# navigator8972/vae_assoc

Measured on AMD Instinct MI355X. Metric: paired-samples/sec (img+jnt assoc-VAE train step), higher is better.
Workload: dtype bf16

## Files before the change

### vae_assoc_amd/csrc/avae_device.h

```cpp
#pragma once
#include <hip/hip_runtime.h>
#include <stdint.h>

namespace avae {

constexpr int kMaxMod = 4;
constexpr int kThreads = 256;
constexpr int kTileBytesK = 128;
constexpr int kRowAlign = 256;
constexpr int kLatentRows = 16;
constexpr int kAdamRows = 16;
constexpr int kCostHist = 4096;

enum Kind : int {
    K_FWD_HIDDEN = 0,
    K_FWD_HEAD = 1,
    K_FWD_OUT_LOSS = 2,
    K_FWD_OUT_STORE = 3,
    K_DGRAD_HIDDEN = 4,
    K_DGRAD_LATENT = 5,
    K_WGRAD = 6,
    K_DGRAD_F32 = 10,
    K_LATENT = 7,
    K_COST = 8,
// ... 28 lines not shown
    void* out2;
    const void* aux0;
    const void* aux1;
    const void* aux2;
    float* partial;
    const float* eps;
    float wts[kMaxMod];
    const void* tail_w;
    void* tail_out;
    const void* tail_aux;
    int tail_mode;
    int tail_n;
    int tail_ldw, tail_ldo, tail_ldx;
    int tail_act;
    int tail_kt;
    int conv;
    const unsigned char* present;
    int present_ld;
};

struct ConvA {
    const void* src;
    const void* consts;
    int M, K;
    int OHW, OW, IH, IW, Cin;
    int k, so, d, pad;
    int src_sb, src_sp;
    int ones;
    unsigned mg_ohw, mg_ow, mg_k, mg_cin;
};
// ... 32 lines not shown
struct TnLaunchArgs {
    int n_items;
    int grid_x;
    int xcd_group;
    int sched;
    int adam;
    long long d_theta, d_m, d_v;
    float beta1, beta2, eps;
    const DevState* st;
    const ConvA* conv_tab;
    int xcd_pieces;
    TnPiece pieces[8][kTnPieces];
    TnItem items[kMaxTnItems];
};
static_assert(sizeof(TnLaunchArgs) <= 4096, "kernel arguments are passed by value: 4 KiB");

struct DevState {
    long long step;
    float last_cost;
    float lr_t;
    float cost_hist[kCostHist];
};

struct AdamItem {
    float* theta;
    float* m;
    float* v;
    const float* g;
    void* W;
    void* Wt;
// ... 216 lines not shown
int tile_lds_bytes(int tile_cfg, bool two_c_tiles);
void launch_grouped(int compute_dtype, int tile_cfg, const LaunchArgs& args, int grid_x, int grid_y, int lds_bytes,
                    DevState* st, hipStream_t s, unsigned long long* stamps = nullptr, int launch_id = 0);
void launch_grouped_tn(int compute_dtype, int tile_cfg, const TnLaunchArgs& args, int grid_x, int grid_y, int lds_bytes,
                       DevState* st, hipStream_t s, unsigned long long* stamps = nullptr, int launch_id = 0);
void launch_adam(int compute_dtype, const AdamArgs& a, int n_blocks, hipStream_t s);
void launch_prep(int compute_dtype, const PrepArgs& a, hipStream_t s);
const void* prep_kernel(int compute_dtype, bool masked);
void launch_fill(void* base, int elem_bytes, unsigned bits, long long start, long long stride, int count, hipStream_t s);
void launch_sums(const ReduceArgs& a, int n_blocks, hipStream_t s);
int small_head_lds_bytes();
void launch_small_latb(int compute_dtype, int act, const LaunchArgs& args, int grid_x, int grid_y, int lds_bytes, DevState* st, hipStream_t s,
                       unsigned long long* stamps, int launch_id);
void launch_small_head(int compute_dtype, int act, const LaunchArgs& args, int grid_x, int grid_y, int lds_bytes, hipStream_t s,
                       unsigned long long* stamps, int launch_id);
void launch_small_tn(int compute_dtype, const TnLaunchArgs& args, int grid_x, int grid_y, hipStream_t s, unsigned long long* stamps, int launch_id);
void launch_small_loss(int compute_dtype, const LaunchArgs& args, int grid_x, int grid_y, int lds_bytes, hipStream_t s, unsigned long long* stamps, int launch_id);
void launch_small(int compute_dtype, const LaunchArgs& args, int grid_x, int grid_y, int lds_bytes, hipStream_t s, unsigned long long* stamps, int launch_id);
void launch_reduce(const ReduceArgs& a, int n_blocks, hipStream_t s);
void launch_chain2(int compute_dtype, const LaunchArgs& args, int grid_x, int grid_y, int lds_bytes, unsigned* counters, unsigned* err, hipStream_t s);

}
```

### vae_assoc_amd/csrc/avae_host.hip

```cpp
#include "avae_device.h"
#include "avae_complete.h"
#include "../../include/avae.h"

#include <dlfcn.h>
#include <sched.h>
#include <unistd.h>

#include <algorithm>
#include <cmath>
#include <cstdio>
#include <cstdlib>
#include <cstring>
#include <functional>
#include <map>
#include <mutex>
#include <stdexcept>
#include <string>
#include <vector>

using namespace avae;

namespace {

thread_local std::string g_create_error;
// ... 154 lines not shown
    size_t P_flat = 0, P_int = 0, P_enc = 0;
    size_t off_theta = 0, off_m = 0, off_v = 0, off_g = 0;
    size_t stage_lo = 0, stage_bytes = 0;
    size_t off_eps = 0, off_partial = 0, off_state = 0, off_items = 0, off_adam = 0, off_inf = 0, off_stamps = 0, off_latent = 0;
    int n_partial = 0;
    size_t ws_bytes = 0;
    unsigned char* ws = nullptr;
    bool own_ws = false;
    hipStream_t cap_stream = nullptr;

    std::vector<WorkItem> items;
    std::vector<Launch> bwd;
    std::vector<Launch> wgrad;
    std::vector<Launch> wgrad_adam;
    int n_buckets = 1;
    int bwd_split = 0;
    std::vector<Launch> wgrad_b[2];
    struct Range { size_t off, count; };
    std::vector<Range> ranges_b[2];
    int adam_first_b[2] = {0, 0}, adam_count_b[2] = {0, 0}, adam_blocks_b[2] = {0, 0};
    std::vector<AdamItem> adam_items_b;
    size_t off_adam_b = 0;
    void* comm = nullptr;
    int comm_world = 1, comm_rank = 0;
    bool comm_on = false;
    size_t off_wire = 0;
    unsigned char* ipc_block = nullptr;
    size_t ipc_bytes = 0;
    unsigned char* ipc_peer[kMaxWorld] = {nullptr, nullptr, nullptr, nullptr, nullptr, nullptr, nullptr, nullptr};
    bool ipc_opened[kMaxWorld] = {false, false, false, false, false, false, false, false};
// ... 941 lines not shown
            bool lean = true;
            int act = -1;
            for (int k = 0; k < Lp.count; ++k) {
                const WorkItem& n = h->items[Lp.first + k];
                if (n.kind == K_COST) continue;
                lean = lean && n.kind == want_p && n.tail_mode == mode
                            && (act < 0 || act == n.tail_act) && n.K > 0 && 2 * n.nz <= 64 && n.tail_kt >= 1 && n.tail_kt <= 2;
                act = n.tail_act;
            }
            if (lean && mode == 1)
                for (int k = 0; k < Lp.count; ++k) lean = lean && h->items[Lp.first + k].kind == K_FWD_HEAD && h->items[Lp.first + k].out1 != nullptr;
            if (lean) { Lp.cfg = mode == 2 ? 10 : 11; Lp.lds = small_head_lds_bytes(); Lp.lean_act = act; }
        }
        return true;
    };
    auto every_conv = [](const Mod&) { return true; };
    auto gather_launch = [&](const std::string& name, std::vector<Launch>& dst, auto&& stage_of, auto&& src_of, auto&& want) {
        Launch L;
        L.name = name; L.type = 1;
        int base = 0;
        for (Mod& md : h->mods) if (md.conv && want(md)) {
            GatherSeg g = bd.gather_seg(stage_of(md), src_of(md));
            g.tile_base = base; base += g.tiles_r * g.tiles_c;
            L.ga.seg[L.ga.n_seg++] = g;
        }
        L.blocks = base;
        if (base > 0) dst.push_back(L);
    };
    auto col2im_launch = [&](const std::string& name, std::vector<Launch>& dst, auto&& stage_of, auto&& prev_of, auto&& want) {
        Launch L;
// ... 60 lines not shown
                      [&](Mod& md) { return h->at<void>(md.cenc[2].Y.rm); }, [](const Mod& md) { return !md.cenc[3].impl; });
    }
    group("fwd_head", h->plain.fwd, [&] { for (Mod& md : h->mods) h->items.push_back(bd.fwd_head(md, true, md.conv && md.cenc[3].impl)); });
    bool latent_alone = false;
    {
        long t64 = 0, t128 = 0;
        bool narrow = false;
        for (const Mod& md : h->mods) {
            t64 += (long)((h->B + 255) / 256) * ((md.n_in + 63) / 64);
            t128 += (long)((h->B + 127) / 128) * ((md.n_in + 127) / 128);
            narrow = narrow || md.n_in <= 64 || h->B <= 64;
        }
        latent_alone = t64 >= 192 && t128 >= 192 && !narrow && !std::getenv("AVAE_NO_LOSS8");
    }
    if (latent_alone) group("latent", h->plain.fwd, [&] { h->items.push_back(bd.latent()); });
    for (int k = 0; k < std::max(Lmax, 1); ++k) {
        group("fwd_dec" + std::to_string(k + 1), h->plain.fwd, [&] {
            for (Mod& md : h->mods) if (k < md.L) h->items.push_back(bd.fwd_hidden(k == 0 ? md.Z : md.D[k - 1], md.dec[k], md.D[k]));
        });
        if (k == 0 && !any_conv && !latent_alone) fuse_tail(h->plain.fwd, 1);
    }
    if (any_conv) {
        Launch L;
        L.name = "conv_wadj"; L.type = 6;
        int base = 0;
        for (Mod& md : h->mods) if (md.conv) for (const ConvStage& st : md.cdec) if (st.adj) {
            WadjSeg& g = L.wa.seg[L.wa.n_seg++];
            g.Wt = h->at<void>(st.d.Wt); g.Wadj = h->at<void>(st.Wadj); g.Wf = h->at<void>(st.Wf); g.ldt = st.d.ldt; g.ldadj = st.ldadj; g.ldf = st.ldf;
            g.k = st.g.k; g.Cin = st.g.Cin; g.Cout = st.d.out;
            g.block_base = base; base += (st.g.Cin * st.g.k * st.g.k * st.d.out + kThreads - 1) / kThreads;
        }
        L.blocks = base;
        if (base > 0 && std::getenv("AVAE_NO_WADJ_FOLD")) h->plain.fwd.push_back(L);
    }
    if (any_conv) {
// ... 84 lines not shown
            if (!md.conv) h->items.push_back(bd.dgrad_latent(md));
            else if (md.cdec[0].impl_bwd) h->items.push_back(bd.adj_dgrad_latent_impl(md.cdec[0], md));
        }
        h->items.push_back(bd.cost(true));
    });
    (void)latent_conv_impl;
    h->bwd_split = (int)h->bwd.size();
    group("bwd_head", h->bwd, [&] {
        for (Mod& md : h->mods) {
            if (md.conv && md.cenc[3].impl_bwd)
                h->items.push_back(bd.adj_dgrad_impl(md.cenc[3], h->at<void>(md.dH.rm), md.dH.ld, md.dH.ld, md.cenc[2].act, md.cenc[2].Y, md.cenc[2].dY));
            else if (md.conv) h->items.push_back(bd.conv_dgrad(md.cenc[3], md.dH));
            else h->items.push_back(bd.dgrad_hidden(md.dH, md.head, md.E.back(), md.dE.back()));
        }
    });
    if (!any_conv) fuse_tail(h->bwd, 2);
    if (any_conv) {
        for (int i = 3; i >= 1; --i) {
            col2im_launch("conv_enc" + std::to_string(i) + "_col2im", h->bwd, [&](Mod& md) -> const ConvStage& { return md.cenc[i]; },
                          [&](Mod& md) -> const ConvStage* { return &md.cenc[i - 1]; }, [i](const Mod& md) { return !md.cenc[i].impl_bwd; });
            if (i >= 2) group("conv_bwd_enc" + std::to_string(i), h->bwd, [&] {
                for (Mod& md : h->mods) if (md.conv) {
                    const ConvStage& st = md.cenc[i - 1];
                    if (st.impl_bwd) h->items.push_back(bd.adj_dgrad_impl(st, h->at<void>(st.dY.rm), st.g.OH * st.g.OW * st.dY.ld, st.dY.ld, md.cenc[i - 2].act, md.cenc[i - 2].Y, md.cenc[i - 2].dY));
                    else h->items.push_back(bd.conv_dgrad(st, st.dY));
                } });
        }
    }
    for (int k = Lmax - 1; k >= 1; --k) {
        group("bwd_enc" + std::to_string(k + 1), h->bwd, [&] {
            for (Mod& md : h->mods) if (k < md.L) h->items.push_back(bd.dgrad_hidden(md.dE[k], md.enc[k], md.E[k - 1], md.dE[k - 1]));
        });
    }
    if (any_conv && !std::getenv("AVAE_NO_SINK")) {
        auto plain_kind = [](int k) { return k == K_FWD_HIDDEN || k == K_DGRAD_HIDDEN || k == K_DGRAD_F32; };
        std::vector<const void*> conv_bufs;
        for (const Mod& md : h->mods) if (md.conv) {
            for (const Act* a : {&md.Z, &md.dH, &md.dO}) conv_bufs.push_back(h->at<void>(a->rm));
            for (const std::vector<ConvStage>* side : {&md.cenc, &md.cdec})
                for (const ConvStage& st : *side) { conv_bufs.push_back(h->at<void>(st.Y.rm)); conv_bufs.push_back(h->at<void>(st.dY.rm)); }
        }
        auto mlp_item = [&](const WorkItem& w) {
            if (w.conv > 0) return false;
            for (const void* q : conv_bufs) if (q == w.out0 || q == w.A) return false;
            return true;
        };
        auto reads = [&](const Launch& L, const std::vector<const void*>& outs) {
            if (L.type != 0) return false;
// ... 439 lines not shown
    return L;
}

void run_launch(avae_handle* h, const Launch& L, hipStream_t s, unsigned long long* stamps, int stamp) {
    Timed t(h, s, L.name);
    if (L.type == 1) launch_gather(h->cfg.compute_dtype, L.ga, L.blocks, s);
    else if (L.type == 2) launch_col2im(h->cfg.compute_dtype, L.ca, L.blocks, s);
    else if (L.type == 3) launch_reduce(L.ra, L.blocks, s);
    else if (L.type == 4) launch_thin(h->cfg.compute_dtype, L.ta, L.blocks, s);
    else if (L.type == 5) launch_colsum(L.ra, L.blocks, s);
    else if (L.type == 6) launch_wadj(h->cfg.compute_dtype, L.wa, L.blocks, s);
    else if (L.type == 7) launch_gperm(L.gp, L.blocks, s);
    else if (L.type == 8) launch_rowsum(h->cfg.compute_dtype, L.rs, L.blocks, s);
    else if (L.type == 9) launch_sums(L.ra, L.blocks, s);
    else if (L.cfg == 13) launch_chain2(h->cfg.compute_dtype, L.args, L.grid_x, L.grid_y, L.lds, h->at<unsigned>(h->off_chain), h->at<unsigned>(h->off_chain) + kMaxMod * 64, s);
    else if (L.cfg == 11) launch_small_head(h->cfg.compute_dtype, L.lean_act, L.args, L.grid_x, L.grid_y, L.lds, s, stamps, stamp);
    else if (L.cfg == 10) launch_small_latb(h->cfg.compute_dtype, L.lean_act, L.args, L.grid_x, L.grid_y, L.lds, h->state(), s, stamps, stamp);
    else if (L.cfg == 9) launch_small_loss(h->cfg.compute_dtype, L.args, L.grid_x, L.grid_y, L.lds, s, stamps, stamp);
    else if (L.cfg == 7) launch_small(h->cfg.compute_dtype, L.args, L.grid_x, L.grid_y, L.lds, s, stamps, stamp);
    else if (L.tn && L.cfg == 12) launch_small_tn(h->cfg.compute_dtype, L.targs, L.grid_x, L.grid_y, s, stamps, stamp);
    else if (L.tn) launch_grouped_tn(h->cfg.compute_dtype, L.cfg, L.targs, L.grid_x, L.grid_y, L.lds, h->state(), s, stamps, stamp);
    else launch_grouped(h->cfg.compute_dtype, L.cfg, L.args, L.grid_x, L.grid_y, L.lds, h->state(), s, stamps, stamp);
    LAUNCH_OK(L.name);
    if (h->debug_sync) {
        std::fprintf(stderr, "[avae] launch %s type=%d cfg=%d items=%d blocks=%d\n", L.name.c_str(), L.type, L.cfg, L.count, L.blocks);
        for (int i = 0; i < L.args.n_items && L.type == 0; ++i)
            std::fprintf(stderr, "        item kind=%d M=%d N=%d K=%d lda=%d ldb=%d tiles=%dx%d\n", L.args.items[i].kind, L.args.items[i].M,
                         L.args.items[i].N, L.args.items[i].K, L.args.items[i].lda, L.args.items[i].ldb, L.args.items[i].tiles_m, L.args.items[i].tiles_n);
        for (int i = 0; i < L.ga.n_seg && L.type == 1; ++i)
            std::fprintf(stderr, "        gather B=%d IH=%d Cin=%d OH=%d k=%d so=%d d=%d pad=%d sb=%d sp=%d ones=%d ldp=%d tiles=%dx%d\n", L.ga.seg[i].g.B, L.ga.seg[i].g.IH,
// ... 396 lines not shown
    bool any_conv = false;
    for (const Mod& md : h->mods) any_conv = any_conv || md.conv;
    out[0].clear(); out[1].clear();
    if (any_conv || h->cfg.comm_buckets == 1) { *n_buckets = 1; out[0].push_back({0, h->P_int + 1}); return; }
    *n_buckets = 2;
    out[1].push_back({0, h->P_enc});
    out[0].push_back({h->P_enc, h->P_int + 1 - h->P_enc});
}

void dp_segment(avae_handle* h, int j, int bucket, hipStream_t s, bool direct = false) {
    if (bucket < 0 || bucket >= h->n_buckets) throw Err("data-parallel bucket out of range");
    if (j < 0 || j >= kMultiSteps) throw Err("staging set out of range");
    auto body = [&](hipStream_t cs) {
        auto run = [&](const std::vector<Launch>& ls, size_t lo, size_t hi) { run_set(h, ls, lo, hi, j, cs); };
        if (h->n_buckets == 1) { run(h->plain.fwd, 0, h->plain.fwd.size()); run(h->bwd, 0, h->bwd.size()); run(h->wgrad, 0, h->wgrad.size()); return; }
        if (bucket == 0) { run(h->plain.fwd, 0, h->plain.fwd.size()); run(h->bwd, 0, (size_t)h->bwd_split); run(h->wgrad_b[0], 0, h->wgrad_b[0].size()); }
        else { run(h->bwd, (size_t)h->bwd_split, h->bwd.size()); run(h->wgrad_b[1], 0, h->wgrad_b[1].size()); }
    };
    if (h->cfg.use_graph && !h->timing && !direct) {
        if (h->g_dp[bucket].empty()) h->g_dp[bucket].resize(kMultiSteps);
        if (!h->g_dp[bucket][j].exec) h->g_dp[bucket][j] = capture(h, body);
        HIP_OK(hipGraphLaunch(h->g_dp[bucket][j].exec, s));
    } else {
        body(s);
    }
}

void dp_allreduce(avae_handle* h, int b, hipStream_t cs) {
    const avae_handle::Range& r = h->ranges_b[b][0];
    float* g = h->grad();
    const bool has_cost = r.off + r.count == h->P_int + 1;
    const size_t n = has_cost ? r.count - 1 : r.count;
// ... 1223 lines not shown
```

### vae_assoc_amd/csrc/avae_kernels.hip

```cpp
#include "avae_device.h"
#include "avae_complete.h"
#include <hip/hip_ext.h>
#include <stdexcept>
#include "../../include/avae.h"

namespace avae {

typedef __attribute__((ext_vector_type(8))) __bf16 bf16x8;
typedef __attribute__((ext_vector_type(4))) __bf16 bf16x4;
typedef __attribute__((ext_vector_type(4))) float f32x4;
typedef __attribute__((ext_vector_type(4))) unsigned u32x4;


template <typename CT> __device__ __forceinline__ CT to_ct(float v);
template <> __device__ __forceinline__ float to_ct<float>(float v) { return v; }
template <> __device__ __forceinline__ __bf16 to_ct<__bf16>(float v) { return (__bf16)v; }

__device__ __forceinline__ float bf16_bits_to_float(unsigned b) { return __uint_as_float(b << 16); }

template <typename CT> __device__ __forceinline__ void load4(const CT* p, float v[4]);
template <> __device__ __forceinline__ void load4<float>(const float* p, float v[4]) {
    float4 t = *reinterpret_cast<const float4*>(p);
    v[0] = t.x; v[1] = t.y; v[2] = t.z; v[3] = t.w;
}
// ... 1673 lines not shown
            default: AVAE_LAUNCH((K_LATB_B(AVAE_ACT_IDENTITY)), grid, block, lds_bytes, s, args, st, stamps, launch_id); break;
        }
    } else {
        switch (act) {
            case AVAE_ACT_RELU: AVAE_LAUNCH((K_LATB_F(AVAE_ACT_RELU)), grid, block, lds_bytes, s, args, st, stamps, launch_id); break;
            case AVAE_ACT_SOFTPLUS: AVAE_LAUNCH((K_LATB_F(AVAE_ACT_SOFTPLUS)), grid, block, lds_bytes, s, args, st, stamps, launch_id); break;
            case AVAE_ACT_SIGMOID: AVAE_LAUNCH((K_LATB_F(AVAE_ACT_SIGMOID)), grid, block, lds_bytes, s, args, st, stamps, launch_id); break;
            case AVAE_ACT_TANH: AVAE_LAUNCH((K_LATB_F(AVAE_ACT_TANH)), grid, block, lds_bytes, s, args, st, stamps, launch_id); break;
            default: AVAE_LAUNCH((K_LATB_F(AVAE_ACT_IDENTITY)), grid, block, lds_bytes, s, args, st, stamps, launch_id); break;
        }
    }
#undef K_LATB_B
#undef K_LATB_F
}

template <typename CT, bool ADAM>
__global__ void __launch_bounds__(kThreads) k_small_tn(const TnLaunchArgs args, unsigned long long* stamps, int launch_id) {
    constexpr int BM = 64, RING = 4, ES = (int)sizeof(CT), EPR = kTileBytesK / ES, NCH = 4;
    constexpr int kStage = 2 * BM * kTileBytesK;
    unsigned char* smem = avae_dyn_smem;
#ifdef AVAE_STAMPS
    unsigned long long sv[kStampWords] = {0, 0, 0, 0, 0, 0, 0, 0};
#endif
    AVAE_STAMP(0)
    const int part = blockIdx.x & 7, idx = blockIdx.x >> 3;
    int entry = blockIdx.y, t_piece = -1;
    if (args.xcd_pieces) {
        const TnPiece* row = args.pieces[part];
        int e = 0, lo = 0;
#pragma unroll
// ... 1783 lines not shown
```

Baseline: 4.763 million.

## Fuse second hidden layer into latent head/dgrad kernels via rider items

Adds k_small_head2 and k_small_latb2 kernels. After the head (forward) or latent-dgrad (backward) tail computes its activation tile, it keeps that tile in LDS and also computes the next hidden layer's GEMM against a prefetched weight panel. The host folds the following fwd_dec2/bwd_enc layer launch into the preceding launch through a 'rider' item index, and keeps an unfused backward list for the bucketed path. This removes one kernel launch and the global round trip of the intermediate activation, at the cost of more LDS per block, redundant tail work across column blocks, and bf16-only constraints.

```diff
diff --git a/vae_assoc_amd/csrc/avae_device.h b/vae_assoc_amd/csrc/avae_device.h
--- a/vae_assoc_amd/csrc/avae_device.h
+++ b/vae_assoc_amd/csrc/avae_device.h
@@ -66,6 +66,7 @@
     int tail_ldw, tail_ldo, tail_ldx;
     int tail_act;
     int tail_kt;
+    int rider;
     int conv;
     const unsigned char* present;
     int present_ld;
@@ -128,6 +129,7 @@
     TnItem items[kMaxTnItems];
 };
 static_assert(sizeof(TnLaunchArgs) <= 4096, "kernel arguments are passed by value: 4 KiB");
+static_assert(sizeof(LaunchArgs) + 24 <= 4096, "kernel arguments are passed by value: 4 KiB");
 
 struct DevState {
     long long step;
@@ -374,6 +376,12 @@
                        unsigned long long* stamps, int launch_id);
 void launch_small_head(int compute_dtype, int act, const LaunchArgs& args, int grid_x, int grid_y, int lds_bytes, hipStream_t s,
                        unsigned long long* stamps, int launch_id);
+int small_head2_max_k();
+int small_head2_lds_bytes(int k_tiles);
+void launch_small_latb2(int compute_dtype, int act, const LaunchArgs& args, int grid_x, int grid_y, int lds_bytes, DevState* st, hipStream_t s,
+                        unsigned long long* stamps, int launch_id);
+void launch_small_head2(int compute_dtype, int act, const LaunchArgs& args, int grid_x, int grid_y, int lds_bytes, hipStream_t s,
+                        unsigned long long* stamps, int launch_id);
 void launch_small_tn(int compute_dtype, const TnLaunchArgs& args, int grid_x, int grid_y, hipStream_t s, unsigned long long* stamps, int launch_id);
 void launch_small_loss(int compute_dtype, const LaunchArgs& args, int grid_x, int grid_y, int lds_bytes, hipStream_t s, unsigned long long* stamps, int launch_id);
 void launch_small(int compute_dtype, const LaunchArgs& args, int grid_x, int grid_y, int lds_bytes, hipStream_t s, unsigned long long* stamps, int launch_id);
diff --git a/vae_assoc_amd/csrc/avae_host.hip b/vae_assoc_amd/csrc/avae_host.hip
--- a/vae_assoc_amd/csrc/avae_host.hip
+++ b/vae_assoc_amd/csrc/avae_host.hip
@@ -192,6 +192,7 @@
     std::vector<Launch> wgrad;
     std::vector<Launch> wgrad_adam;
     int n_buckets = 1;
+    std::vector<Launch> bwd_b;
     int bwd_split = 0;
     std::vector<Launch> wgrad_b[2];
     struct Range { size_t off, count; };
@@ -1163,6 +1164,48 @@
         }
         return true;
     };
+    auto fuse_tail2 = [&](std::vector<Launch>& ls, int mode) {
+        if (ls.size() < 2 || std::getenv("AVAE_NO_TAIL2") || h->cfg.compute_dtype != AVAE_BF16) return false;
+        Launch& Lp = ls[ls.size() - 2];
+        Launch& Lc = ls[ls.size() - 1];
+        if (Lp.type != 0 || Lc.type != 0 || Lp.tn || Lc.tn || Lp.cfg != (mode == 2 ? 10 : 11) || Lc.cfg != 7) return false;
+        for (const Mod& md : h->mods) if (md.conv || md.L < 2) return false;
+        const int want_p = mode == 1 ? K_FWD_HEAD : K_DGRAD_LATENT, want_c = mode == 1 ? K_FWD_HIDDEN : K_DGRAD_HIDDEN;
+        int n_prod = 0;
+        for (int k = 0; k < Lp.count; ++k) n_prod += Lp.args.items[k].kind == want_p ? 1 : 0;
+        if (Lc.count != n_prod || Lp.count + Lc.count > kMaxItemsPerLaunch) return false;
+        std::vector<int> prod(Lc.count, -1);
+        int k_tiles = 0;
+        for (int i = 0; i < Lc.count; ++i) {
+            const WorkItem& c = Lc.args.items[i];
+            if (c.kind != want_c || c.act != Lp.lean_act || c.bias_ep || c.conv || c.N > 1024 || c.K > small_head2_max_k()) return false;
+            for (int k = 0; k < Lp.count; ++k) {
+                const WorkItem& n = Lp.args.items[k];
+                if (n.kind != want_p || n.tail_mode != mode || n.rider || n.M != c.M || n.tail_kt != 1) continue;
+                if (n.tail_out == c.A && n.tail_ldo == c.lda && c.K == (int)rup(n.tail_n + (mode == 1 ? 1 : 0), h->KU)) {
+                    bool taken = false;
+                    for (int j = 0; j < i; ++j) taken = taken || prod[j] == k;
+                    if (!taken) prod[i] = k;
+                }
+            }
+            if (prod[i] < 0) return false;
+            k_tiles = std::max(k_tiles, c.K / h->KU);
+        }
+        const int lds = small_head2_lds_bytes(k_tiles);
+        if (lds > 160 * 1024) return false;
+        for (int i = 0; i < Lc.count; ++i) {
+            const WorkItem c = Lc.args.items[i];
+            Lp.args.items[Lp.count + i] = c;
+            for (WorkItem* n : {&h->items[Lp.first + prod[i]], &Lp.args.items[prod[i]]}) { n->rider = Lp.count + i + 1; n->tiles_n = c.tiles_n; }
+        }
+        Lp.args.n_items = Lp.count + Lc.count;
+        int max_tiles = 1;
+        for (int k = 0; k < Lp.count; ++k) max_tiles = std::max(max_tiles, Lp.args.items[k].tiles_m * Lp.args.items[k].tiles_n);
+        Lp.grid_x = (max_tiles + 7) & ~7; Lp.blocks = Lp.grid_x * Lp.grid_y; Lp.args.grid_x = Lp.grid_x;
+        Lp.cfg = mode == 2 ? 14 : 15; Lp.lds = lds;
+        ls.pop_back();
+        return true;
+    };
     auto every_conv = [](const Mod&) { return true; };
     auto gather_launch = [&](const std::string& name, std::vector<Launch>& dst, auto&& stage_of, auto&& src_of, auto&& want) {
         Launch L;
@@ -1253,11 +1296,13 @@
         latent_alone = t64 >= 192 && t128 >= 192 && !narrow && !std::getenv("AVAE_NO_LOSS8");
     }
     if (latent_alone) group("latent", h->plain.fwd, [&] { h->items.push_back(bd.latent()); });
+    bool tail_fwd = false;
     for (int k = 0; k < std::max(Lmax, 1); ++k) {
         group("fwd_dec" + std::to_string(k + 1), h->plain.fwd, [&] {
             for (Mod& md : h->mods) if (k < md.L) h->items.push_back(bd.fwd_hidden(k == 0 ? md.Z : md.D[k - 1], md.dec[k], md.D[k]));
         });
-        if (k == 0 && !any_conv && !latent_alone) fuse_tail(h->plain.fwd, 1);
+        if (k == 0 && !any_conv && !latent_alone) tail_fwd = fuse_tail(h->plain.fwd, 1);
+        if (k == 1 && tail_fwd) fuse_tail2(h->plain.fwd, 1);
     }
     if (any_conv) {
         Launch L;
@@ -1372,7 +1417,7 @@
             else h->items.push_back(bd.dgrad_hidden(md.dH, md.head, md.E.back(), md.dE.back()));
         }
     });
-    if (!any_conv) fuse_tail(h->bwd, 2);
+    const bool tail_bwd = !any_conv && fuse_tail(h->bwd, 2);
     if (any_conv) {
         for (int i = 3; i >= 1; --i) {
             col2im_launch("conv_enc" + std::to_string(i) + "_col2im", h->bwd, [&](Mod& md) -> const ConvStage& { return md.cenc[i]; },
@@ -1385,11 +1430,18 @@
                 } });
         }
     }
+    h->bwd_b.clear();
     for (int k = Lmax - 1; k >= 1; --k) {
         group("bwd_enc" + std::to_string(k + 1), h->bwd, [&] {
             for (Mod& md : h->mods) if (k < md.L) h->items.push_back(bd.dgrad_hidden(md.dE[k], md.enc[k], md.E[k - 1], md.dE[k - 1]));
         });
-    }
+        if (k == Lmax - 1 && tail_bwd) {
+            const std::vector<Launch> unfused = h->bwd;
+            if (fuse_tail2(h->bwd, 2)) h->bwd_b = unfused;
+        }
+    }
+    if (!h->bwd_b.empty())
+        for (size_t i = h->bwd_b.size() - 1; i < h->bwd.size(); ++i) h->bwd_b.push_back(h->bwd[i]);
     if (any_conv && !std::getenv("AVAE_NO_SINK")) {
         auto plain_kind = [](int k) { return k == K_FWD_HIDDEN || k == K_DGRAD_HIDDEN || k == K_DGRAD_F32; };
         std::vector<const void*> conv_bufs;
@@ -1859,6 +1911,8 @@
     else if (L.type == 8) launch_rowsum(h->cfg.compute_dtype, L.rs, L.blocks, s);
     else if (L.type == 9) launch_sums(L.ra, L.blocks, s);
     else if (L.cfg == 13) launch_chain2(h->cfg.compute_dtype, L.args, L.grid_x, L.grid_y, L.lds, h->at<unsigned>(h->off_chain), h->at<unsigned>(h->off_chain) + kMaxMod * 64, s);
+    else if (L.cfg == 15) launch_small_head2(h->cfg.compute_dtype, L.lean_act, L.args, L.grid_x, L.grid_y, L.lds, s, stamps, stamp);
+    else if (L.cfg == 14) launch_small_latb2(h->cfg.compute_dtype, L.lean_act, L.args, L.grid_x, L.grid_y, L.lds, h->state(), s, stamps, stamp);
     else if (L.cfg == 11) launch_small_head(h->cfg.compute_dtype, L.lean_act, L.args, L.grid_x, L.grid_y, L.lds, s, stamps, stamp);
     else if (L.cfg == 10) launch_small_latb(h->cfg.compute_dtype, L.lean_act, L.args, L.grid_x, L.grid_y, L.lds, h->state(), s, stamps, stamp);
     else if (L.cfg == 9) launch_small_loss(h->cfg.compute_dtype, L.args, L.grid_x, L.grid_y, L.lds, s, stamps, stamp);
@@ -2285,8 +2339,9 @@
     auto body = [&](hipStream_t cs) {
         auto run = [&](const std::vector<Launch>& ls, size_t lo, size_t hi) { run_set(h, ls, lo, hi, j, cs); };
         if (h->n_buckets == 1) { run(h->plain.fwd, 0, h->plain.fwd.size()); run(h->bwd, 0, h->bwd.size()); run(h->wgrad, 0, h->wgrad.size()); return; }
-        if (bucket == 0) { run(h->plain.fwd, 0, h->plain.fwd.size()); run(h->bwd, 0, (size_t)h->bwd_split); run(h->wgrad_b[0], 0, h->wgrad_b[0].size()); }
-        else { run(h->bwd, (size_t)h->bwd_split, h->bwd.size()); run(h->wgrad_b[1], 0, h->wgrad_b[1].size()); }
+        const std::vector<Launch>& bw = h->bwd_b.empty() ? h->bwd : h->bwd_b;
+        if (bucket == 0) { run(h->plain.fwd, 0, h->plain.fwd.size()); run(bw, 0, (size_t)h->bwd_split); run(h->wgrad_b[0], 0, h->wgrad_b[0].size()); }
+        else { run(bw, (size_t)h->bwd_split, bw.size()); run(h->wgrad_b[1], 0, h->wgrad_b[1].size()); }
     };
     if (h->cfg.use_graph && !h->timing && !direct) {
         if (h->g_dp[bucket].empty()) h->g_dp[bucket].resize(kMultiSteps);
diff --git a/vae_assoc_amd/csrc/avae_kernels.hip b/vae_assoc_amd/csrc/avae_kernels.hip
--- a/vae_assoc_amd/csrc/avae_kernels.hip
+++ b/vae_assoc_amd/csrc/avae_kernels.hip
@@ -1711,6 +1711,428 @@
 #undef K_LATB_F
 }
 
+constexpr int kT2Blocks = 8;
+constexpr int kT2Tiles = 4 * kT2Blocks * 16 * 2 / kTileBytesK;
+constexpr int kT2Tile = 32 * kTileBytesK;
+int small_head2_max_k() { return 4 * kT2Blocks * 16; }
+int small_head2_lds_bytes(int k_tiles) { return small_head_lds_bytes() + 2 * k_tiles * kT2Tile; }
+
+__device__ __forceinline__ void t2_put4(unsigned char* aimg, int row, int c0, const float v[4]) {
+    const int bo = (c0 & 63) * 2;
+    const uint2 pk = {pack_bf16(v[0], v[1]), pack_bf16(v[2], v[3])};
+    *reinterpret_cast<uint2*>(aimg + (c0 >> 6) * kT2Tile + row * kTileBytesK + ((((bo >> 4) ^ ((row >> 1) & 7)) << 4) | (bo & 15))) = pk;
+}
+__device__ __forceinline__ f32x4 t2_tile(const unsigned char* aimg, const unsigned char* panel, int nk, int wr, int wc, int fr, int fq) {
+    const int sw0 = (fq ^ (fr >> 1)) * 16;
+    const int aoff = (wr * 16 + fr) * kTileBytesK, boff = (wc * 16 + fr) * kTileBytesK;
+    f32x4 acc = {0.f, 0.f, 0.f, 0.f};
+    for (int kt = 0; kt < nk; ++kt) {
+        const unsigned char* Sa = aimg + kt * kT2Tile + aoff;
+        const unsigned char* Sp = panel + kt * kT2Tile + boff;
+        const u32x4 a0 = *reinterpret_cast<const u32x4*>(Sa + sw0), b0 = *reinterpret_cast<const u32x4*>(Sp + sw0);
+        const u32x4 a1 = *reinterpret_cast<const u32x4*>(Sa + (sw0 ^ 64)), b1 = *reinterpret_cast<const u32x4*>(Sp + (sw0 ^ 64));
+        mma<__bf16>(b0, a0, acc);
+        mma<__bf16>(b1, a1, acc);
+    }
+    return acc;
+}
+
+template <int ACT>
+__global__ void __launch_bounds__(kThreads) k_small_head2(const LaunchArgs args, unsigned long long* stamps, int launch_id) {
+    typedef __bf16 CT;
+    constexpr int RING = 4, ES = 2, LDM = 68, NCB = kT2Blocks;
+    unsigned char* smem = avae_dyn_smem;
+    unsigned char* img = smem + RING * kHeadStage;
+    unsigned char* aimg = img + kHeadImg + 64;
+    float* MV = reinterpret_cast<float*>(smem);
+#ifdef AVAE_STAMPS
+    unsigned long long sv[kStampWords] = {0, 0, 0, 0, 0, 0, 0, 0};
+#endif
+    AVAE_STAMP(0)
+    const int part = blockIdx.x & 7, idx = blockIdx.x >> 3;
+    const WorkItem w = args.items[blockIdx.y];
+    const WorkItem& rd = args.items[w.rider - 1];
+    const void* rB = rd.B;
+    CT* rout = reinterpret_cast<CT*>(rd.out0);
+    const int rK = rd.K, rN = rd.N, rldb = rd.ldb, rld0 = rd.ld0;
+    asm volatile("" :: "s"(w.A), "s"(w.B), "s"(w.out0), "s"(w.out1), "s"(w.aux0), "s"(w.lda), "s"(w.ldb), "s"(w.K), "s"(w.ld0), "s"(w.tail_w), "s"(w.tail_out));
+    asm volatile("" :: "s"(rB), "s"(rout), "s"(rK), "s"(rN), "s"(rldb), "s"(rld0));
+    int t;
+    {
+        const int nt = w.tiles_m * w.tiles_n;
+        const int q = nt >> 3, r = nt & 7;
+        if (idx >= q + (part < r ? 1 : 0)) return;
+        t = (part < r ? part * (q + 1) : r * (q + 1) + (part - r) * q) + idx;
+    }
+    const int tid = threadIdx.x, lane = tid & 63, wave = __builtin_amdgcn_readfirstlane(tid >> 6);
+    const int wr = wave >> 1, wc = wave & 1, fr = lane & 15, fq = lane >> 4;
+    const int tm = t / w.tiles_n, cb = t - tm * w.tiles_n;
+    const int m0 = tm * 32;
+    const int nk = (w.K * ES) / kTileBytesK, nz = w.nz, nk2 = (rK * ES) / kTileBytesK;
+    unsigned char* panel = aimg + nk2 * kT2Tile;
+    typedef const __attribute__((address_space(1))) void* gp_t;
+    typedef __attribute__((address_space(3))) void* lp_t;
+    reinterpret_cast<f32x4*>(img)[tid] = f32x4{0.f, 0.f, 0.f, 0.f};
+    reinterpret_cast<f32x4*>(img)[tid + kThreads] = f32x4{0.f, 0.f, 0.f, 0.f};
+    const int zrow = tid >> 3, zg = tid & 7;
+    const f32x4 ev = *reinterpret_cast<const f32x4*>(reinterpret_cast<const float*>(w.aux0) + (size_t)min(m0 + zrow, w.M - 1) * w.ldx + min(4 * zg, w.ldx - 4));
+    const int prow = wave * 8 + (lane >> 3), lc = ((lane & 7) ^ ((prow >> 1) & 7)) * 16;
+    const unsigned char* srcA = reinterpret_cast<const unsigned char*>(w.A) + (size_t)(m0 + prow) * w.lda * ES + lc;
+    const unsigned char* srcB = reinterpret_cast<const unsigned char*>(w.B) + (size_t)prow * w.ldb * ES + lc;
+    const unsigned char* srcP = reinterpret_cast<const unsigned char*>(rB) + (size_t)(cb * 32 + prow) * rldb * ES + lc;
+    const size_t b32 = (size_t)32 * w.ldb * ES;
+#define AVAE_H_DMA(kt, buf)                                                                                             \
+    { __builtin_amdgcn_global_load_lds((gp_t)(srcA + (size_t)(kt) * kTileBytesK), (lp_t)(smem + (buf) * kHeadStage + wave * 1024), 16, 0, 0);       \
+      __builtin_amdgcn_global_load_lds((gp_t)(srcB + (size_t)(kt) * kTileBytesK), (lp_t)(smem + (buf) * kHeadStage + (4 + wave) * 1024), 16, 0, 0); \
+      __builtin_amdgcn_global_load_lds((gp_t)(srcB + b32 + (size_t)(kt) * kTileBytesK), (lp_t)(smem + (buf) * kHeadStage + (8 + wave) * 1024), 16, 0, 0); }
+    AVAE_STAMP(1)
+    const int npro = nk < RING - 1 ? nk : RING - 1;
+    for (int p = 0; p < npro; ++p) AVAE_H_DMA(p, p)
+    constexpr int kExtra = 2 * NCB + kT2Tiles;
+    asm volatile("" ::: "memory"); __builtin_amdgcn_sched_barrier(0);
+    u32x4 tb[NCB][2];
+#pragma unroll
+    for (int i = 0; i < NCB; ++i) {
+        const unsigned char* pw = reinterpret_cast<const unsigned char*>(w.tail_w) + (size_t)min(16 * (4 * i + wave) + fr, w.tail_n - 1) * w.tail_ldw * ES + fq * 16;
+        tb[i][0] = *reinterpret_cast<const u32x4*>(pw);
+        tb[i][1] = *reinterpret_cast<const u32x4*>(pw + 64);
+    }
+#pragma unroll
+    for (int kt = 0; kt < kT2Tiles; ++kt) {
+        const int ktc = min(kt, nk2 - 1);
+        __builtin_amdgcn_global_load_lds((gp_t)(srcP + (size_t)ktc * kTileBytesK), (lp_t)(panel + ktc * kT2Tile + wave * 1024), 16, 0, 0);
+    }
+    asm volatile("" ::: "memory"); __builtin_amdgcn_sched_barrier(0);
+    const int sw0 = (fq ^ (fr >> 1)) * 16;
+    const int aoff = (wr * 16 + fr) * kTileBytesK, boff = (32 + wc * 32 + fr) * kTileBytesK;
+    f32x4 acc[2] = {{0.f, 0.f, 0.f, 0.f}, {0.f, 0.f, 0.f, 0.f}};
+    int buf = 0;
+    for (int kt = 0; kt < nk; ++kt) {
+        const int rem = nk - 1 - kt;
+        if (kt < npro) {
+            if (rem >= 2) asm volatile("s_waitcnt vmcnt(%0)" :: "n"(6 + kExtra) : "memory");
+            else if (rem == 1) asm volatile("s_waitcnt vmcnt(%0)" :: "n"(3 + kExtra) : "memory");
+            else asm volatile("s_waitcnt vmcnt(%0)" :: "n"(kExtra) : "memory");
+        } else {
+            if (rem >= 2) asm volatile("s_waitcnt vmcnt(6)" ::: "memory");
+            else if (rem == 1) asm volatile("s_waitcnt vmcnt(3)" ::: "memory");
+            else asm volatile("s_waitcnt vmcnt(0)" ::: "memory");
+        }
+        asm volatile("s_barrier" ::: "memory");
+        if (kt == 0) { AVAE_STAMP(2) }
+        const unsigned char* Sb = smem + buf * kHeadStage;
+        const u32x4 a0 = *reinterpret_cast<const u32x4*>(Sb + aoff + sw0);
+        const u32x4 b00 = *reinterpret_cast<const u32x4*>(Sb + boff + sw0), b01 = *reinterpret_cast<const u32x4*>(Sb + boff + 16 * kTileBytesK + sw0);
+        const int fill = buf == 0 ? RING - 1 : buf - 1;
+        if (kt + RING - 1 < nk) AVAE_H_DMA(kt + RING - 1, fill)
+        const u32x4 a1 = *reinterpret_cast<const u32x4*>(Sb + aoff + (sw0 ^ 64));
+        const u32x4 b10 = *reinterpret_cast<const u32x4*>(Sb + boff + (sw0 ^ 64)), b11 = *reinterpret_cast<const u32x4*>(Sb + boff + 16 * kTileBytesK + (sw0 ^ 64));
+        mma<CT>(b00, a0, acc[0]); mma<CT>(b01, a0, acc[1]);
+        mma<CT>(b10, a1, acc[0]); mma<CT>(b11, a1, acc[1]);
+        buf = buf + 1 == RING ? 0 : buf + 1;
+    }
+#undef AVAE_H_DMA
+#pragma unroll
+    for (int i = 0; i < NCB; ++i) asm volatile("" :: "v"(tb[i][0]), "v"(tb[i][1]));
+    asm volatile("s_waitcnt vmcnt(0)" ::: "memory");
+    lds_barrier();
+    AVAE_STAMP(3)
+    {
+        const int orow = m0 + wr * 16 + fr, lrow = wr * 16 + fr;
+        float* mulv = reinterpret_cast<float*>(w.out0) + (size_t)orow * w.ld0;
+        const bool store = cb == 0 && orow < w.M;
+#pragma unroll
+        for (int j = 0; j < 2; ++j) {
+            const int c0 = wc * 32 + j * 16 + 4 * fq;
+            *reinterpret_cast<f32x4*>(MV + lrow * LDM + c0) = acc[j];
+            if (store) {
+#pragma unroll
+                for (int e = 0; e < 4; ++e) if (c0 + e < 2 * nz) mulv[c0 + e] = acc[j][e];
+            }
+        }
+    }
+    lds_barrier();
+    AVAE_STAMP(5)
+    {
+        CT* Z = reinterpret_cast<CT*>(w.out1) + (size_t)(m0 + zrow) * w.ld1;
+        const bool store = cb == 0 && m0 + zrow < w.M;
+#pragma unroll
+        for (int e = 0; e < 4; ++e) {
+            const int d = 4 * zg + e;
+            if (d < nz) {
+                const float z = __builtin_fmaf(fexp(0.5f * MV[zrow * LDM + nz + d]), ev[e], MV[zrow * LDM + d]);
+                img_put<CT>(img, zrow, d, z);
+                if (store) Z[d] = to_ct<CT>(z);
+            }
+        }
+        if (tid < 32) img_put<CT>(img, tid, nz, 1.0f);
+    }
+    lds_barrier();
+    {
+        u32x4 ta[2][2];
+#pragma unroll
+        for (int rh = 0; rh < 2; ++rh)
+#pragma unroll
+            for (int sl = 0; sl < 2; ++sl) {
+                const int arow = 16 * rh + fr;
+                ta[rh][sl] = *reinterpret_cast<const u32x4*>(img + arow * kTileBytesK + (((fq + 4 * sl) ^ ((arow >> 1) & 7)) << 4));
+            }
+        unsigned own = 0;
+        for (int b = cb; b < 4 * NCB; b += w.tiles_n) own |= 1u << b;
+        CT* D1 = reinterpret_cast<CT*>(w.tail_out);
+        const int H1 = w.tail_n;
+#pragma unroll
+        for (int i = 0; i < NCB; ++i) {
+            const int b = 4 * i + wave, c0 = 16 * b + 4 * fq;
+            if (16 * b < rK) {
+#pragma unroll
+                for (int rh = 0; rh < 2; ++rh) {
+                    f32x4 ta_acc = {0.f, 0.f, 0.f, 0.f};
+                    mma<CT>(tb[i][0], ta[rh][0], ta_acc);
+                    mma<CT>(tb[i][1], ta[rh][1], ta_acc);
+                    const int row = 16 * rh + fr;
+                    float v[4];
+#pragma unroll
+                    for (int e = 0; e < 4; ++e) v[e] = c0 + e < H1 ? act_fwd_t<ACT>(ta_acc[e]) : (c0 + e == H1 ? 1.0f : 0.0f);
+                    t2_put4(aimg, row, c0, v);
+                    if (((own >> b) & 1u) && m0 + row < w.M && c0 < H1) store_row<CT>(D1 + (size_t)(m0 + row) * w.tail_ldo + c0, v, H1 - c0);
+                }
+            }
+        }
+    }
+    lds_barrier();
+    AVAE_STAMP_EP(6)
+    {
+        const f32x4 c = t2_tile(aimg, panel, nk2, wr, wc, fr, fq);
+        const int orow = m0 + wr * 16 + fr, ocol = cb * 32 + wc * 16 + 4 * fq;
+        if (orow < w.M && ocol < rN) {
+            float v[4];
+#pragma unroll
+            for (int e = 0; e < 4; ++e) v[e] = act_fwd_t<ACT>(c[e]);
+            store_row<CT>(rout + (size_t)orow * rld0 + ocol, v, rN - ocol);
+        }
+    }
+    AVAE_STAMP(4)
+    AVAE_STAMP_FLUSH()
+}
+
+template <int ACT>
+__global__ void __launch_bounds__(kThreads) k_small_latb2(const LaunchArgs args, DevState* st, unsigned long long* stamps, int launch_id) {
+    typedef __bf16 CT;
+    constexpr int RING = 4, ES = 2, NCB = kT2Blocks;
+    unsigned char* smem = avae_dyn_smem;
+    unsigned char* img = smem + RING * kHeadStage;
+    float* red = reinterpret_cast<float*>(img + kHeadImg);
+    unsigned char* aimg = img + kHeadImg + 64;
+#ifdef AVAE_STAMPS
+    unsigned long long sv[kStampWords] = {0, 0, 0, 0, 0, 0, 0, 0};
+#endif
+    AVAE_STAMP(0)
+    const int part = blockIdx.x & 7, idx = blockIdx.x >> 3;
+    const WorkItem w = args.items[blockIdx.y];
+    asm volatile("" :: "s"(w.A), "s"(w.B), "s"(w.out0), "s"(w.aux2), "s"(w.lda), "s"(w.ldb), "s"(w.K), "s"(w.ld0), "s"(w.tail_w), "s"(w.tail_out), "s"(w.tail_aux));
+    int t;
+    {
+        const int nt = w.tiles_m * w.tiles_n;
+        const int q = nt >> 3, r = nt & 7;
+        if (idx >= q + (part < r ? 1 : 0)) return;
+        t = (part < r ? part * (q + 1) : r * (q + 1) + (part - r) * q) + idx;
+    }
+    if (w.kind == K_COST) {
+        cost_item<4>(w, st, red);
+        AVAE_STAMP(4)
+        AVAE_STAMP_FLUSH()
+        return;
+    }
+    const WorkItem& rd = args.items[w.rider - 1];
+    const void* rB = rd.B;
+    const CT* raux = reinterpret_cast<const CT*>(rd.aux0);
+    CT* rout = reinterpret_cast<CT*>(rd.out0);
+    const int rK = rd.K, rN = rd.N, rldb = rd.ldb, rld0 = rd.ld0, rldx = rd.ldx;
+    asm volatile("" :: "s"(rB), "s"(raux), "s"(rout), "s"(rK), "s"(rN), "s"(rldb), "s"(rld0), "s"(rldx));
+    const int tid = threadIdx.x, lane = tid & 63, wave = __builtin_amdgcn_readfirstlane(tid >> 6);
+    const int wr = wave >> 1, wc = wave & 1, fr = lane & 15, fq = lane >> 4;
+    const int tm = t / w.tiles_n, cb = t - tm * w.tiles_n;
+    const int m0 = tm * 32;
+    const int nk = (w.K * ES) / kTileBytesK, nz = w.nz, nk2 = (rK * ES) / kTileBytesK;
+    unsigned char* panel = aimg + nk2 * kT2Tile;
+    typedef const __attribute__((address_space(1))) void* gp_t;
+    typedef __attribute__((address_space(3))) void* lp_t;
+    reinterpret_cast<f32x4*>(img)[tid] = f32x4{0.f, 0.f, 0.f, 0.f};
+    reinterpret_cast<f32x4*>(img)[tid + kThreads] = f32x4{0.f, 0.f, 0.f, 0.f};
+    const int orow = m0 + wr * 16 + fr;
+    const int lde = (nz + 3) & ~3;
+    const int prow = wave * 8 + (lane >> 3), lc = ((lane & 7) ^ ((prow >> 1) & 7)) * 16;
+    const unsigned char* srcA = reinterpret_cast<const unsigned char*>(w.A) + (size_t)(m0 + prow) * w.lda * ES + lc;
+    const unsigned char* srcB = reinterpret_cast<const unsigned char*>(w.B) + (size_t)prow * w.ldb * ES + lc;
+    const unsigned char* srcP = reinterpret_cast<const unsigned char*>(rB) + (size_t)(cb * 32 + prow) * rldb * ES + lc;
+    const size_t b32 = (size_t)32 * w.ldb * ES;
+#define AVAE_H_DMA(kt, buf)                                                                                             \
+    { __builtin_amdgcn_global_load_lds((gp_t)(srcA + (size_t)(kt) * kTileBytesK), (lp_t)(smem + (buf) * kHeadStage + wave * 1024), 16, 0, 0);       \
+      __builtin_amdgcn_global_load_lds((gp_t)(srcB + (size_t)(kt) * kTileBytesK), (lp_t)(smem + (buf) * kHeadStage + (4 + wave) * 1024), 16, 0, 0); \
+      __builtin_amdgcn_global_load_lds((gp_t)(srcB + b32 + (size_t)(kt) * kTileBytesK), (lp_t)(smem + (buf) * kHeadStage + (8 + wave) * 1024), 16, 0, 0); }
+    AVAE_STAMP(1)
+    const int npro = nk < RING - 1 ? nk : RING - 1;
+    for (int p = 0; p < npro; ++p) AVAE_H_DMA(p, p)
+    constexpr int kExtra = 6 + 2 * NCB + 2 * NCB + 1 + kT2Tiles;
+    static_assert(6 + kExtra <= 63, "vmcnt is a 6-bit counter");
+    asm volatile("" ::: "memory"); __builtin_amdgcn_sched_barrier(0);
+    f32x4 gm[2], gl[2], gf[2];
+#pragma unroll
+    for (int j = 0; j < 2; ++j) {
+        const float* gr = reinterpret_cast<const float*>(w.aux2) + (size_t)min(orow, w.M - 1) * 3 * lde + min(wc * 32 + j * 16 + 4 * fq, lde - 4);
+        gm[j] = *reinterpret_cast<const f32x4*>(gr); gl[j] = *reinterpret_cast<const f32x4*>(gr + lde); gf[j] = *reinterpret_cast<const f32x4*>(gr + 2 * lde);
+    }
+    u32x4 tb[NCB][2];
+    uint2 ty[NCB][2];
+#pragma unroll
+    for (int i = 0; i < NCB; ++i) {
+        const int b = 4 * i + wave;
+        const unsigned char* pw = reinterpret_cast<const unsigned char*>(w.tail_w) + (size_t)min(16 * b + fr, w.tail_n - 1) * w.tail_ldw * ES + fq * 16;
+        tb[i][0] = *reinterpret_cast<const u32x4*>(pw);
+        tb[i][1] = *reinterpret_cast<const u32x4*>(pw + 64);
+#pragma unroll
+        for (int rh = 0; rh < 2; ++rh)
+            ty[i][rh] = *reinterpret_cast<const uint2*>(reinterpret_cast<const CT*>(w.tail_aux) + (size_t)min(m0 + 16 * rh + fr, w.M - 1) * w.tail_ldx
+                                                        + min(16 * b + 4 * fq, w.tail_ldx - 4));
+    }
+    const int ocol = cb * 32 + wc * 16 + 4 * fq;
+    const uint2 yq = *reinterpret_cast<const uint2*>(raux + (size_t)min(orow, w.M - 1) * rldx + min(ocol, rldx - 4));
+#pragma unroll
+    for (int kt = 0; kt < kT2Tiles; ++kt) {
+        const int ktc = min(kt, nk2 - 1);
+        __builtin_amdgcn_global_load_lds((gp_t)(srcP + (size_t)ktc * kTileBytesK), (lp_t)(panel + ktc * kT2Tile + wave * 1024), 16, 0, 0);
+    }
+    asm volatile("" ::: "memory"); __builtin_amdgcn_sched_barrier(0);
+    const int sw0 = (fq ^ (fr >> 1)) * 16;
+    const int aoff = (wr * 16 + fr) * kTileBytesK, boff = (32 + wc * 32 + fr) * kTileBytesK;
+    f32x4 acc[2] = {{0.f, 0.f, 0.f, 0.f}, {0.f, 0.f, 0.f, 0.f}};
+    int buf = 0;
+    for (int kt = 0; kt < nk; ++kt) {
+        const int rem = nk - 1 - kt;
+        if (kt < npro) {
+            if (rem >= 2) asm volatile("s_waitcnt vmcnt(%0)" :: "n"(6 + kExtra) : "memory");
+            else if (rem == 1) asm volatile("s_waitcnt vmcnt(%0)" :: "n"(3 + kExtra) : "memory");
+            else asm volatile("s_waitcnt vmcnt(%0)" :: "n"(kExtra) : "memory");
+        } else {
+            if (rem >= 2) asm volatile("s_waitcnt vmcnt(6)" ::: "memory");
+            else if (rem == 1) asm volatile("s_waitcnt vmcnt(3)" ::: "memory");
+            else asm volatile("s_waitcnt vmcnt(0)" ::: "memory");
+        }
+        asm volatile("s_barrier" ::: "memory");
+        if (kt == 0) { AVAE_STAMP(2) }
+        const unsigned char* Sb = smem + buf * kHeadStage;
+        const u32x4 a0 = *reinterpret_cast<const u32x4*>(Sb + aoff + sw0);
+        const u32x4 b00 = *reinterpret_cast<const u32x4*>(Sb + boff + sw0), b01 = *reinterpret_cast<const u32x4*>(Sb + boff + 16 * kTileBytesK + sw0);
+        const int fill = buf == 0 ? RING - 1 : buf - 1;
+        if (kt + RING - 1 < nk) AVAE_H_DMA(kt + RING - 1, fill)
+        const u32x4 a1 = *reinterpret_cast<const u32x4*>(Sb + aoff + (sw0 ^ 64));
+        const u32x4 b10 = *reinterpret_cast<const u32x4*>(Sb + boff + (sw0 ^ 64)), b11 = *reinterpret_cast<const u32x4*>(Sb + boff + 16 * kTileBytesK + (sw0 ^ 64));
+        mma<CT>(b00, a0, acc[0]); mma<CT>(b01, a0, acc[1]);
+        mma<CT>(b10, a1, acc[0]); mma<CT>(b11, a1, acc[1]);
+        buf = buf + 1 == RING ? 0 : buf + 1;
+    }
+#undef AVAE_H_DMA
+#pragma unroll
+    for (int i = 0; i < NCB; ++i) asm volatile("" :: "v"(tb[i][0]), "v"(tb[i][1]), "v"(ty[i][0]), "v"(ty[i][1]));
+    asm volatile("" :: "v"(yq), "v"(gm[0]), "v"(gm[1]), "v"(gl[0]), "v"(gl[1]), "v"(gf[0]), "v"(gf[1]));
+    asm volatile("s_waitcnt vmcnt(0)" ::: "memory");
+    AVAE_STAMP(3)
+    {
+        CT* dH = reinterpret_cast<CT*>(w.out0) + (size_t)orow * w.ld0;
+        const bool store = cb == 0 && orow < w.M;
+        const int lrow = wr * 16 + fr;
+#pragma unroll
+        for (int j = 0; j < 2; ++j)
+#pragma unroll
+            for (int e = 0; e < 4; ++e) {
+                const int d = wc * 32 + j * 16 + 4 * fq + e;
+                if (d < nz) {
+                    const float dz = acc[j][e];
+                    const float dmu = dz + gm[j][e], dlv = __builtin_fmaf(dz, gf[j][e], gl[j][e]);
+                    img_put<CT>(img, lrow, d, dmu);
+                    img_put<CT>(img, lrow, nz + d, dlv);
+                    if (store) { dH[d] = to_ct<CT>(dmu); dH[nz + d] = to_ct<CT>(dlv); }
+                }
+            }
+    }
+    lds_barrier();
+    AVAE_STAMP(5)
+    {
+        u32x4 ta[2][2];
+#pragma unroll
+        for (int rh = 0; rh < 2; ++rh)
+#pragma unroll
+            for (int sl = 0; sl < 2; ++sl) {
+                const int arow = 16 * rh + fr;
+                ta[rh][sl] = *reinterpret_cast<const u32x4*>(img + arow * kTileBytesK + (((fq + 4 * sl) ^ ((arow >> 1) & 7)) << 4));
+            }
+        unsigned own = 0;
+        for (int b = cb; b < 4 * NCB; b += w.tiles_n) own |= 1u << b;
+        CT* dE = reinterpret_cast<CT*>(w.tail_out);
+        const int H = w.tail_n;
+#pragma unroll
+        for (int i = 0; i < NCB; ++i) {
+            const int b = 4 * i + wave, c0 = 16 * b + 4 * fq;
+            if (16 * b < rK) {
+#pragma unroll
+                for (int rh = 0; rh < 2; ++rh) {
+                    f32x4 ta_acc = {0.f, 0.f, 0.f, 0.f};
+                    mma<CT>(tb[i][0], ta[rh][0], ta_acc);
+                    mma<CT>(tb[i][1], ta[rh][1], ta_acc);
+                    const int row = 16 * rh + fr;
+                    float v[4];
+#pragma unroll
+                    for (int e = 0; e < 4; ++e) v[e] = c0 + e < H ? ta_acc[e] * act_bwd_t<ACT>(quad_elem<CT>(ty[i][rh], e)) : 0.0f;
+                    t2_put4(aimg, row, c0, v);
+                    if (((own >> b) & 1u) && m0 + row < w.M && c0 < H) store_row<CT>(dE + (size_t)(m0 + row) * w.tail_ldo + c0, v, H - c0);
+                }
+            }
+        }
+    }
+    lds_barrier();
+    AVAE_STAMP_EP(6)
+    {
+        const f32x4 c = t2_tile(aimg, panel, nk2, wr, wc, fr, fq);
+        if (orow < w.M && ocol < rN) {
+            float v[4];
+#pragma unroll
+            for (int e = 0; e < 4; ++e) v[e] = c[e] * act_bwd_t<ACT>(quad_elem<CT>(yq, e));
+            store_row<CT>(rout + (size_t)orow * rld0 + ocol, v, rN - ocol);
+        }
+    }
+    AVAE_STAMP(4)
+    AVAE_STAMP_FLUSH()
+}
+
+#define AVAE_T2_DISPATCH(KERNEL, ...)                                                                                    \
+    static const bool once = [] {                         \
+        set_max_lds(KERNEL<AVAE_ACT_RELU>); set_max_lds(KERNEL<AVAE_ACT_SOFTPLUS>); set_max_lds(KERNEL<AVAE_ACT_SIGMOID>);  \
+        set_max_lds(KERNEL<AVAE_ACT_TANH>); set_max_lds(KERNEL<AVAE_ACT_IDENTITY>);                                        \
+        return true;                                                                                                     \
+    }();                                                                                                                 \
+    (void)once;                                                                                                          \
+    switch (act) {                                                                                                       \
+        case AVAE_ACT_RELU: AVAE_LAUNCH((KERNEL<AVAE_ACT_RELU>), grid, block, lds_bytes, s, __VA_ARGS__); break;         \
+        case AVAE_ACT_SOFTPLUS: AVAE_LAUNCH((KERNEL<AVAE_ACT_SOFTPLUS>), grid, block, lds_bytes, s, __VA_ARGS__); break; \
+        case AVAE_ACT_SIGMOID: AVAE_LAUNCH((KERNEL<AVAE_ACT_SIGMOID>), grid, block, lds_bytes, s, __VA_ARGS__); break;   \
+        case AVAE_ACT_TANH: AVAE_LAUNCH((KERNEL<AVAE_ACT_TANH>), grid, block, lds_bytes, s, __VA_ARGS__); break;         \
+        default: AVAE_LAUNCH((KERNEL<AVAE_ACT_IDENTITY>), grid, block, lds_bytes, s, __VA_ARGS__); break;                \
+    }
+void launch_small_head2(int compute_dtype, int act, const LaunchArgs& args, int grid_x, int grid_y, int lds_bytes, hipStream_t s,
+                        unsigned long long* stamps, int launch_id) {
+    if (compute_dtype != AVAE_BF16) throw std::runtime_error("internal error: the second tail runs in bf16 only");
+    const dim3 grid(grid_x, grid_y), block(kThreads);
+    AVAE_T2_DISPATCH(k_small_head2, args, stamps, launch_id)
+}
+void launch_small_latb2(int compute_dtype, int act, const LaunchArgs& args, int grid_x, int grid_y, int lds_bytes, DevState* st, hipStream_t s,
+                        unsigned long long* stamps, int launch_id) {
+    if (compute_dtype != AVAE_BF16) throw std::runtime_error("internal error: the second tail runs in bf16 only");
+    const dim3 grid(grid_x, grid_y), block(kThreads);
+    AVAE_T2_DISPATCH(k_small_latb2, args, st, stamps, launch_id)
+}
+#undef AVAE_T2_DISPATCH
+
 template <typename CT, bool ADAM>
 __global__ void __launch_bounds__(kThreads) k_small_tn(const TnLaunchArgs args, unsigned long long* stamps, int launch_id) {
     constexpr int BM = 64, RING = 4, ES = (int)sizeof(CT), EPR = kTileBytesK / ES, NCH = 4;
```

Measured after the change: 4.392 million. 0.922x the previous value.
